# janelia-flyem/flypylib

Measured on AMD Instinct MI355X. Metric: inference Mvoxels/sec, vgg_like (rf 18, 22^3 coarse -> 88^3 per reference tile), synthetic EM uint8 volume, higher is better.
Workload: dtype f16s; 1 GPU; the 520^3 volume of BASELINE.json's metric (configs[0]'s substack size) per GPU: vgg_like inference, 520x520x520 synthetic uint8 volume, reference tile lattice 102^3 (pitch 88), u8 in / f32 out resident in HBM; tile_in=102, executor=vgg_split_f16, parallelism=z-slab tile sharding x1, no collective, device=AMD Radeon Graphics (gfx950:sramecc+:xnack-)

## Files before the change

flypylib_amd/csrc/vgg_plan.h:

```cpp
#pragma once
#include <algorithm>
#include <cstdint>
#include <vector>

struct VggSlab {
  int64_t VZ, VY, VX;
  int64_t fz_hi;
  int64_t cz_lo, cz_hi;
  int CY, CX;
  bool empty;
};

static inline VggSlab vgg_slab(const int64_t dims[3], const std::vector<int32_t> &origins_z,
                               int32_t out_sz_z, int32_t zb, int32_t ze, int off) {
  VggSlab s = {};
  s.VZ = dims[0] - 2 * off; s.VY = dims[1] - 2 * off; s.VX = dims[2] - 2 * off;
  s.empty = s.VZ <= 0 || s.VY <= 0 || s.VX <= 0 || zb >= ze;
  if (s.empty) return s;
  const int64_t fz_lo = (int64_t)origins_z[zb] - off;
  s.fz_hi = std::min<int64_t>((int64_t)origins_z[ze - 1] - off + out_sz_z, s.VZ);
  s.cz_lo = fz_lo / 4; s.cz_hi = (s.fz_hi + 3) / 4;
  s.CY = (int)((s.VY + 3) / 4); s.CX = (int)((s.VX + 3) / 4);
  return s;
}

struct VggPyramid {
  int P2, P1;
  explicit VggPyramid(int64_t C) : P2((int)C + 2), P1(2 * P2 + 2) {}
};
struct Vgg2Pyramid {
  int Q, T3, H;
  explicit Vgg2Pyramid(int64_t C) : Q((int)C + 2), T3(2 * Q + 2), H(T3 + 2) {}
};

static inline int64_t vgg_chunk_rows(int64_t budget_bytes, int64_t bytes_per_fine_row,
                                     int fixed_rows, int64_t span, int64_t cap = 0) {
  int64_t c = std::max<int64_t>(4, (budget_bytes / bytes_per_fine_row - fixed_rows) / 2);
  c = std::min<int64_t>(c, span);
  c = (c + 3) / 4 * 4;
  return cap ? std::min<int64_t>(c, cap) : c;
}

static inline int64_t vgg_split_max_p1_rows(int P1Y, int P1X, int tile_z) {
  return ((int64_t)1 << 32) / 16 / ((int64_t)P1Y * P1X) - (tile_z + 2);
}
static inline int64_t vgg_split_chunk_cap(int64_t max_rows) {
  return std::max<int64_t>(4, ((max_rows - VggPyramid(0).P1) / 2) / 4 * 4);
}

enum { MID_INTERIOR = 0, MID_XCOL = 1, MID_ZLAYER = 2 };

struct MidGeo {
  int BZ, BY, BX;
  int ZS;
  constexpr int TZ() const { return BZ + 2; }
  constexpr int TY() const { return BY + 2; }
  constexpr int TX() const { return BX + 2; }
  constexpr int slots() const { return (TZ() - 1) * ZS + TY() * TX(); }
  constexpr int slot(int tz, int ty, int tx) const { return tz * ZS + ty * TX() + tx; }
};
constexpr MidGeo mid_geo(int o) {
  return o == MID_XCOL ? MidGeo{8, 16, 4, 108} : o == MID_ZLAYER ? MidGeo{4, 8, 16, 182} : MidGeo{8, 4, 16, 118};
}

struct MidVox { int z, y, x; };
constexpr MidVox mid_voxel(int o, int wave, int sub, int c) {
  return o == MID_XCOL     ? MidVox{2 * (wave >> 1) + (sub >> 1), c, 2 * (wave & 1) + (sub & 1)}
         : o == MID_ZLAYER ? MidVox{2 * (wave >> 2) + (sub >> 1), 2 * (wave & 3) + (sub & 1), c}
                           : MidVox{2 * (wave >> 1) + (sub >> 1), 2 * (wave & 1) + (sub & 1), c};
}
constexpr MidVox mid_slot_voxel(const MidGeo &g, int s) {
  const int tz = s / g.ZS < g.TZ() ? s / g.ZS : g.TZ() - 1;
  const int rem = s - tz * g.ZS < g.TY() * g.TX() ? s - tz * g.ZS : g.TY() * g.TX() - 1;
  return MidVox{tz, rem / g.TX(), rem % g.TX()};
}
constexpr int mid_tap_slot(const MidGeo &g, int tap) { return g.slot(tap / 9, (tap / 3) % 3, tap % 3); }

struct MidWalk {
  int nbx, nby, nbz;
  int z0, x0;
  constexpr int64_t blocks() const { return (int64_t)nbx * nby * nbz; }
};
struct MidPlan { MidWalk w[3]; };

static inline MidPlan vgg_mid_plan(int Z, int Y, int X, bool reorient) {
  auto cdiv = [](int a, int b) { return (a + b - 1) / b; };
  const MidGeo gi = mid_geo(MID_INTERIOR), gx = mid_geo(MID_XCOL), gz = mid_geo(MID_ZLAYER);
  MidPlan p = {};
  MidWalk &in = p.w[MID_INTERIOR], &xc = p.w[MID_XCOL], &zl = p.w[MID_ZLAYER];
  in = MidWalk{cdiv(2 * X, gi.BX), cdiv(2 * Y, gi.BY), cdiv(2 * Z, gi.BZ), 0, 0};
  if (!reorient) return p;
  const int live_x = 2 * X % gi.BX, live_z = 2 * Z % gi.BZ;
  if (live_x) {
    const MidWalk c = {cdiv(live_x, gx.BX), cdiv(2 * Y, gx.BY), cdiv(2 * Z, gx.BZ), 0, (in.nbx - 1) * gi.BX};
    if (c.blocks() < (int64_t)in.nby * in.nbz) { xc = c; --in.nbx; }
  }
  if (live_z && in.nbx) {
    const MidWalk c = {in.nbx, cdiv(2 * Y, gz.BY), cdiv(live_z, gz.BZ), (in.nbz - 1) * gi.BZ, 0};
    if (c.blocks() < (int64_t)in.nbx * in.nby) { zl = c; --in.nbz; }
  }
  return p;
}
```

flypylib_amd/csrc/vgg_split.hip:

```cpp
#define FPL_F16 1
#include <algorithm>
#include <cmath>
#include <initializer_list>

#include "fast_paths.h"
#include "mfma_util.h"
#include "pack_weights.h"
#include "vgg_plan.h"
#include <type_traits>
#include "vgg_split_lds.h"
#include "vgg_tiles.h"

namespace {

constexpr int CH = 48;
constexpr int CHP = 24, NPASS = CH / CHP;
constexpr int LO_OFF = CHP * 2;
constexpr int PASS_BYTES = 2 * LO_OFF;
constexpr int VOX = NPASS * PASS_BYTES;
constexpr int KS = (27 * CHP + 31) / 32;
constexpr int KTAB = (KS + 4) / 4 * 4;
constexpr int KTAB_BYTES = 4 * KTAB * 4;
static_assert(CHP % 8 == 0, "a lane's 8 k-slots stay inside one tap");

__host__ __device__ constexpr int64_t chan_off(int ch, int64_t plane) { return (ch / CHP) * plane + (ch % CHP) * 2; }

__device__ __forceinline__ h16x8 pack_relu_split_x(const f32x4 &blk) {
  u32x4 v;
  Pair2 p;
  p = split_pk_relu(blk[0], blk[1]); v[0] = p.hi; v[2] = p.lo;
  p = split_pk_relu(blk[2], blk[3]); v[1] = p.hi; v[3] = p.lo;
  return __builtin_bit_cast(h16x8, v);
}
__device__ __forceinline__ h16x8 pack_relu_split_x(const f32x4 &blk, unsigned &ovf) {
  const h16x8 r = pack_relu_split_x(blk);
  const u32x4 v = __builtin_bit_cast(u32x4, r);
  ovf_note(ovf, pk_max_i16(v[0], v[1]));
  return r;
}

__device__ __forceinline__ f32x4 chain48(const h16x8 (&w)[4], const Frag2 &h01, h16x8 hx, f32x4 acc) {
  acc = mfma16(w[1], h01.hi, acc);
  acc = mfma16(w[0], h01.lo, acc);
  acc = mfma16(w[2], hx, acc);
  acc = mfma16(w[3], hx, acc);
  return mfma16(w[0], h01.hi, acc);
}

__device__ __forceinline__ void store_split12(unsigned char *vox, int64_t plane, int g, const f32x4 (&v)[3],
                                              unsigned &ovf) {
  unsigned hi[6], lo[6];
#pragma unroll
  for (int b = 0; b < 3; ++b) {
    const Pair2 p0 = split_pk(v[b][0], v[b][1], ovf), p1 = split_pk(v[b][2], v[b][3], ovf);
    hi[2 * b] = p0.hi; hi[2 * b + 1] = p1.hi;
    lo[2 * b] = p0.lo; lo[2 * b + 1] = p1.lo;
  }
  unsigned char *d = vox + (g >> 1) * plane + 24 * (g & 1);
  *reinterpret_cast<u32x4_a8 *>(d) = u32x4_a8{hi[0], hi[1], hi[2], hi[3]};
  *reinterpret_cast<u32x2 *>(d + 16) = u32x2{hi[4], hi[5]};
  *reinterpret_cast<u32x4_a8 *>(d + LO_OFF) = u32x4_a8{lo[0], lo[1], lo[2], lo[3]};
  *reinterpret_cast<u32x2 *>(d + LO_OFF + 16) = u32x2{lo[4], lo[5]};
}

constexpr int S_PZ = 4, S_PY = 8, S_PX = 32;
constexpr int S_TZ = 2 * S_PZ + 2, S_TY = 2 * S_PY + 2, S_TX = 2 * S_PX + 2;
constexpr int S_TP = 80;
constexpr int S_TILE = S_TZ * S_TY * S_TP;
constexpr int S_WAVES = 8;
constexpr int S_ROWS = S_TZ * S_TY;
constexpr int S_WROWS = (S_ROWS + S_WAVES - 1) / S_WAVES;
constexpr int S_TASKS = S_PZ * S_PY * 2 / S_WAVES;
constexpr int S_RPT = 3;
static_assert(S_RPT * S_TASKS >= S_WROWS && S_WROWS <= 64, "stem fill schedule");
constexpr int S_SHTAB = 64 * 48;
constexpr int S_SH2 = 4 * 12;
constexpr int S_SMEM = 4 * S_TILE * 2 + 256 * 4 + S_SHTAB * 4 + 2 * S_SH2 * 4;

struct StemSArgs {
  const void *src;
  int64_t SZ, SY, SX;
  int64_t z_hi;
  float mean, sd;
  float c0;
  const float *shtab;
  int64_t p1z0;
  const h16x8 *w1, *w2;
  const float *shift1, *shift2;
  x8::Tensor p1;
  int nbx, nby, nbz;
  int trim;
  unsigned *flag;
  float xlim;
  unsigned char *dump;
};

__device__ __forceinline__ int stem_row_off(int row) {
  return ((row / 3) * S_TY + row % 3) * S_TP;
}

struct StemBlock {
  int px0, py0, pz0;
  int64_t gz0, gy0, gx0;
  unsigned xc;
  bool x_ok;
};

__device__ __forceinline__ StemBlock stem_block(const StemSArgs &a, int q, int lane) {
  StemBlock b;
  const int xb = q % a.nbx, t = q / a.nbx;
  const int yb = t % a.nby, zb = t / a.nby;
  b.px0 = xb * S_PX; b.py0 = yb * S_PY; b.pz0 = zb * S_PZ;
  b.gz0 = 2 * (a.p1z0 + b.pz0); b.gy0 = 2 * (int64_t)b.py0; b.gx0 = 2 * (int64_t)b.px0;
  const int64_t x = b.gx0 + lane;
  b.x_ok = x < a.SX;
  b.xc = (unsigned)(b.x_ok ? x : a.SX - 1);
  return b;
}

__device__ __forceinline__ int stem_row_of(int wrow0, int l) {
  const int r = wrow0 + (l < S_WROWS ? l : S_WROWS - 1);
  return r < S_ROWS ? r : S_ROWS - 1;
}

template <typename SRC>
__device__ __forceinline__ unsigned stem_row_tab(const StemSArgs &a, const StemBlock &b, int wrow0,
                                                 int lane, const SRC *&base) {
  const int row = stem_row_of(wrow0, lane);
  const int64_t z = b.gz0 + row / S_TY, y = b.gy0 + row % S_TY;
  const bool ok = z < a.z_hi && y < a.SY;
  const int64_t zc = z < a.z_hi ? z : a.z_hi - 1, yc = y < a.SY ? y : a.SY - 1;
  const int64_t zb = b.gz0 < a.z_hi ? b.gz0 : a.z_hi - 1, yb = b.gy0 < a.SY ? b.gy0 : a.SY - 1;
  base = (const SRC *)a.src + (zb * a.SY + yb) * a.SX;
  const unsigned rel = (unsigned)(((zc - zb) * a.SY + (yc - yb)) * a.SX);
  return rel | (ok ? 0x80000000u : 0u);
}

template <typename SRC>
struct StemRows {
  SRC v[S_RPT];
  bool ok[S_RPT];
};

template <typename SRC>
__device__ __forceinline__ void stem_load_rows(const SRC *base, unsigned tab, unsigned xc,
                                               int idx0, StemRows<SRC> &r) {
#pragma unroll
  for (int k = 0; k < S_RPT; ++k) {
    const int idx = idx0 + k < S_WROWS ? idx0 + k : S_WROWS - 1;
    const unsigned t = (unsigned)__builtin_amdgcn_readlane((int)tab, idx);
    r.ok[k] = (t >> 31) != 0u;
    r.v[k] = (base + (t & 0x7FFFFFFFu))[xc];
  }
}

template <typename SRC>
__device__ __forceinline__ unsigned stem_norm(const StemSArgs &a, const unsigned *lut, SRC v,
                                              bool ok, unsigned &xmax) {
  unsigned t;
  if (sizeof(SRC) == 1) {
    t = lut[(unsigned)v & 255u];
  } else {
    const float x = ((float)v - a.mean) / a.sd;
    const unsigned ax = __builtin_bit_cast(unsigned, x) & 0x7FFFFFFFu;
    xmax = ax > xmax ? ax : xmax;
    const h16_t h = (h16_t)x;
    t = (unsigned)h16_bits(x) | ((unsigned)h16_bits(x - (float)h) << 16);
  }
  return ok ? t : 0u;
}

struct StemBits { unsigned b[S_RPT]; };

template <typename SRC>
__device__ __forceinline__ void stem_convert_rows(const StemSArgs &a, const StemBlock &b,
                                                  const unsigned *lut, const StemRows<SRC> &r,
                                                  StemBits &o, unsigned &xmax) {
#pragma unroll
  for (int k = 0; k < S_RPT; ++k) o.b[k] = stem_norm<SRC>(a, lut, r.v[k], r.ok[k] && b.x_ok, xmax);
}

template <bool LO>
__device__ __forceinline__ void stem_write_rows(unsigned short *tile, int wrow0, int idx0, int lane,
                                                const StemBits &o) {
#pragma unroll
  for (int k = 0; k < S_RPT; ++k) {
    const int e = stem_row_of(wrow0, idx0 + k) * S_TP + lane;
    tile[e] = (unsigned short)o.b[k];
    if (LO) tile[S_TILE + e] = (unsigned short)(o.b[k] >> 16);
  }
}

template <typename SRC>
struct StemEdge { SRC v[2]; bool ok[2]; };

template <typename SRC>
__device__ __forceinline__ void stem_load_edge(const StemSArgs &a, const StemBlock &b, int wrow0,
                                               int lane, StemEdge<SRC> &e) {
  const int row = stem_row_of(wrow0, lane);
  const int64_t z = b.gz0 + row / S_TY, y = b.gy0 + row % S_TY;
  const bool rok = z < a.z_hi && y < a.SY;
  const int64_t zc = z < a.z_hi ? z : a.z_hi - 1, yc = y < a.SY ? y : a.SY - 1;
  const SRC *rp = (const SRC *)a.src + (zc * a.SY + yc) * a.SX;
#pragma unroll
  for (int j = 0; j < 2; ++j) {
    const int64_t x = b.gx0 + 64 + j;
    e.ok[j] = rok && x < a.SX;
    e.v[j] = rp[x < a.SX ? x : a.SX - 1];
  }
}

template <typename SRC>
__device__ __forceinline__ void stem_store_edge(const StemSArgs &a, unsigned short *tile,
                                                const unsigned *lut, int wrow0, int lane,
                                                const StemEdge<SRC> &e, unsigned &xmax) {
  const int row = stem_row_of(wrow0, lane);
  const unsigned v0 = stem_norm<SRC>(a, lut, e.v[0], e.ok[0], xmax);
  const unsigned v1 = stem_norm<SRC>(a, lut, e.v[1], e.ok[1], xmax);
  *reinterpret_cast<unsigned *>(&tile[row * S_TP + 64]) = (v0 & 0xFFFFu) | (v1 << 16);
  if (sizeof(SRC) != 1)
    *reinterpret_cast<unsigned *>(&tile[S_TILE + row * S_TP + 64]) = (v0 >> 16) | (v1 & 0xFFFF0000u);
}

struct StemTrim {
  int pxs;
  int ntx, nty;
  int nt;
  int mag;
};

__device__ __forceinline__ StemTrim stem_trim(const StemSArgs &a, const StemBlock &b) {
  StemTrim t;
  const int lx = min(S_PX, a.p1.X - b.px0), ly = min(S_PY, a.p1.Y - b.py0), lz = min(S_PZ, a.p1.Z - b.pz0);
  t.pxs = lx > 8 ? 4 : lx > 4 ? 3 : 2;
  const int pyh = 16 >> t.pxs;
  t.ntx = (lx + (1 << t.pxs) - 1) >> t.pxs;
  t.nty = (ly + pyh - 1) / pyh;
  t.nt = lz * t.nty * t.ntx;
  t.mag = (1024 + t.nty - 1) / t.nty;
  return t;
}

__device__ __forceinline__ bool stem_full(const StemSArgs &a, const StemBlock &b) {
  return b.px0 + S_PX <= a.p1.X && b.py0 + S_PY <= a.p1.Y && b.pz0 + S_PZ <= a.p1.Z;
}

extern __shared__ __attribute__((aligned(16))) unsigned char smem[];

template <typename SRC>
__global__ __launch_bounds__(64 * S_WAVES, 2) void vggs_stem_pool(StemSArgs a) {
  unsigned short *tiles = reinterpret_cast<unsigned short *>(smem);
  unsigned *lut = reinterpret_cast<unsigned *>(smem + 4 * S_TILE * 2);
  const int tid = threadIdx.x, lane = tid & 63;
  const int wave = __builtin_amdgcn_readfirstlane(tid >> 6);
  const int c = lane & 15, g = lane >> 4;
  const int nblocks = a.nbx * a.nby * a.nbz;
  int q = blockIdx.x;
  if (q >= nblocks) return;
  constexpr bool INT = sizeof(SRC) == 1;
  if (INT && tid < 256) lut[tid] = (unsigned)h16_bits((float)tid - a.c0);
  const unsigned char *shtab = smem + 4 * S_TILE * 2 + 256 * 4;
  if (INT)
    for (int i = tid; i < S_SHTAB; i += 64 * S_WAVES)
      reinterpret_cast<float *>(smem + 4 * S_TILE * 2 + 256 * 4)[i] = a.shtab[i];

  int offP[2][3], offS[2][2];
#pragma unroll
  for (int e = 0; e < 2; ++e) {
#pragma unroll
    for (int i = 0; i < 3; ++i)
      offP[e][i] = 2 * (g < 3 ? stem_row_off(3 * g + i) + (e == 0 ? 0 : 2)
                              : stem_row_off(6 + i) + (e == 0 ? 2 : 0));
#pragma unroll
    for (int h = 0; h < 2; ++h)
      offS[e][h] = 2 * (stem_row_off(2 * (g < 3 ? g : 2) + h) + (e == 0 ? 2 : 1));
  }
  h16x8 w1[2][2][3], w2[4][3];
  float *sh2t = reinterpret_cast<float *>(smem + 4 * S_TILE * 2 + 256 * 4 + S_SHTAB * 4);
  if (tid < S_SH2) {
    const float v = a.shift2[x8::out_channel((tid % 12) / 4, tid / 12, tid % 4)];
    sh2t[tid] = v;
    sh2t[S_SH2 + tid] = -v;
  }
  const f32x4 *sh2g = reinterpret_cast<const f32x4 *>(sh2t + 12 * g);
  const f32x4 *sh2n = reinterpret_cast<const f32x4 *>(sh2t + S_SH2 + 12 * g);
  f32x4 sh1[3];
#pragma unroll
  for (int p = 0; p < 2; ++p)
#pragma unroll
    for (int s = 0; s < 2; ++s)
#pragma unroll
      for (int b = 0; b < 3; ++b) {
        w1[p][s][b] = a.w1[((p * 2 + s) * 3 + b) * 64 + lane];
        w2[2 * p + s][b] = a.w2[((2 * p + s) * 3 + b) * 64 + lane];
      }
#pragma unroll
  for (int b = 0; b < 3; ++b)
#pragma unroll
    for (int r = 0; r < 4; ++r) {
      sh1[b][r] = a.shift1[16 * b + 4 * g + r];
    }
  __syncthreads();

  unsigned ovf = 0u, xmax = 0u;
  const int wrow0 = wave * S_WROWS;
  StemBlock blk = stem_block(a, q, lane);
  {
    const SRC *base0;
    const unsigned tab0 = stem_row_tab<SRC>(a, blk, wrow0, lane, base0);
    for (int i0 = 0; i0 < S_WROWS; i0 += S_RPT) {
      StemRows<SRC> rr;
      StemBits hb;
      stem_load_rows<SRC>(base0, tab0, blk.xc, i0, rr);
      stem_convert_rows<SRC>(a, blk, lut, rr, hb, xmax);
      stem_write_rows<!INT>(tiles, wrow0, i0, lane, hb);
    }
    StemEdge<SRC> ee;
    stem_load_edge<SRC>(a, blk, wrow0, lane, ee);
    stem_store_edge<SRC>(a, tiles, lut, wrow0, lane, ee, xmax);
  }
  __syncthreads();

  const int G = (int)gridDim.x;
  auto clampq = [&](int qq, int qlast) { return qq < nblocks ? qq : qlast; };
  StemRows<SRC> rr;
  StemEdge<SRC> ee;
  StemBits hb;
  {
    const StemBlock n0 = stem_block(a, clampq(q + G, q), lane);
    const SRC *bn;
    const unsigned tn = stem_row_tab<SRC>(a, n0, wrow0, lane, bn);
    stem_load_rows<SRC>(bn, tn, n0.xc, 0, rr);
    stem_load_edge<SRC>(a, n0, wrow0, lane, ee);
    stem_convert_rows<SRC>(a, n0, lut, rr, hb, xmax);
    stem_load_rows<SRC>(bn, tn, n0.xc, S_RPT, rr);
    const f32x4 z3[3] = {{0.f, 0.f, 0.f, 0.f}, {0.f, 0.f, 0.f, 0.f}, {0.f, 0.f, 0.f, 0.f}};
    __builtin_amdgcn_sched_barrier(0);
    x8::store12_sel(a.p1, 0, g, z3, ovf, false, a.dump);
  }
  struct Gin {
    unsigned p[INT ? 1 : 2][3], s0[INT ? 1 : 2], s1[INT ? 1 : 2];
  };
  struct Geo { int base, xrel, yrel, zrel, pzl, pyl, pxl; bool live; };
  int cur = 0;
  for (;;) {
    const int qn = q + G;
    const bool has_next = qn < nblocks;
    const StemBlock nxt = stem_block(a, has_next ? qn : q, lane);
    const StemBlock nx2 = stem_block(a, clampq(qn + G, has_next ? qn : q), lane);
    const SRC *base_n, *base_2;
    const unsigned tab_n = stem_row_tab<SRC>(a, nxt, wrow0, lane, base_n);
    const unsigned tab_2 = stem_row_tab<SRC>(a, nx2, wrow0, lane, base_2);
    const unsigned char *tb = reinterpret_cast<const unsigned char *>(tiles + cur * 2 * S_TILE);
    unsigned short *tnext = tiles + (cur ^ 1) * 2 * S_TILE;
    auto geo = [&](int ti) {
      Geo t;
      const int task = wave + S_WAVES * ti;
      const int row = task >> 1;
      const int xh = task & 1;
      t.pzl = row / S_PY; t.pyl = row % S_PY; t.pxl = 16 * xh + c; t.live = true;
      t.base = 2 * (((2 * t.pzl) * S_TY + 2 * t.pyl) * S_TP + 2 * (16 * xh + c));
      t.xrel = (int)(blk.gx0 + 2 * (16 * xh + c) + 3 - a.SX);
      t.yrel = (int)(blk.gy0 + 2 * t.pyl + 3 - a.SY);
      t.zrel = (int)(blk.gz0 + 2 * t.pzl + 3 - a.z_hi);
      return t;
    };
    const StemTrim trm = stem_trim(a, blk);
    auto geo_trim = [&](int ti) {
      Geo t;
      int task = wave + S_WAVES * ti;
      t.live = task < trm.nt;
      task = t.live ? task : trm.nt - 1;
      const int r = task >> (trm.ntx - 1), tx = task & (trm.ntx - 1);
      const int tz = (r * trm.mag) >> 10, ty = r - tz * trm.nty;
      t.pzl = tz;
      t.pyl = (ty << (4 - trm.pxs)) + (c >> trm.pxs);
      t.pxl = (tx << trm.pxs) + (c & ((1 << trm.pxs) - 1));
      t.base = 2 * (((2 * t.pzl) * S_TY + 2 * t.pyl) * S_TP + 2 * t.pxl);
      t.xrel = (int)(blk.gx0 + 2 * t.pxl + 3 - a.SX);
      t.yrel = (int)(blk.gy0 + 2 * t.pyl + 3 - a.SY);
      t.zrel = (int)(blk.gz0 + 2 * t.pzl + 3 - a.z_hi);
      return t;
    };
    const bool interior = INT && blk.gx0 + 2 * S_PX + 2 <= a.SX && blk.gy0 + 2 * S_PY + 2 <= a.SY &&
                          blk.gz0 + 2 * S_PZ + 2 <= a.z_hi;
    auto block_pass = [&](auto edge_t, auto trim_t) {
      constexpr bool EDGE = decltype(edge_t)::value, TRIM = decltype(trim_t)::value;
      auto gg = [&](int ti) {
        if constexpr (TRIM) return geo_trim(ti);
        else return geo(ti);
      };
      const int ntask = TRIM ? max(1, (trm.nt - wave + S_WAVES - 1) / S_WAVES) : S_TASKS;
      f32x4 kin[3];
      if (INT && !EDGE) {
#pragma unroll
        for (int b = 0; b < 3; ++b) kin[b] = *reinterpret_cast<const f32x4 *>(shtab + (4 * g) * 4 + 64 * b);
      }
      auto gather = [&](const Geo &t, int sub, Gin &o) {
        const int sp = sub >> 1, e = sub & 1;
        const int so = 2 * ((((sp >> 1) & 1) * S_TY + (sp & 1)) * S_TP);
#pragma unroll
        for (int part = 0; part < (INT ? 1 : 2); ++part) {
          const unsigned char *tp = tb + part * (S_TILE * 2) + t.base + so;
#pragma unroll
          for (int i = 0; i < 3; ++i) o.p[part][i] = *reinterpret_cast<const unsigned *>(tp + offP[e][i]);
          o.s0[part] = *reinterpret_cast<const unsigned short *>(tp + offS[e][0]);
          o.s1[part] = *reinterpret_cast<const unsigned short *>(tp + offS[e][1]);
        }
      };
      auto gather_init = [&](const Geo &t, int sub, f32x4 (&o)[3]) {
        if (INT && EDGE) {
          const int sp = sub >> 1, e = sub & 1;
          const int pzy = 4 * min(max(t.zrel + (sp >> 1), 0), 3) + min(max(t.yrel + (sp & 1), 0), 3);
          const unsigned char *tp = shtab + ((4 * pzy + min(max(t.xrel + e, 0), 3)) * 48 + 4 * g) * 4;
#pragma unroll
          for (int b = 0; b < 3; ++b) o[b] = *reinterpret_cast<const f32x4 *>(tp + 64 * b);
        }
      };
      auto frag = [&](const Gin &gi, int part) {
        const u32x4 raw = {gi.p[part][0], gi.p[part][1], gi.p[part][2], gi.s0[part] | (gi.s1[part] << 16)};
        return __builtin_bit_cast(h16x8, raw);
      };
      constexpr int NC3 = INT ? 6 : 9;
      auto c3 = [&](int i, int e, const f32x4 (&gin)[3], h16x8 bh, h16x8 bl, f32x4 (&o)[3]) {
        const int b = i % 3, grp = i / 3;
        if (grp == 0) o[b] = mfma16(w1[1][e][b], bh, INT ? (EDGE ? gin[b] : kin[b]) : sh1[b]);
        else if (!INT && grp == 1) o[b] = mfma16(w1[0][e][b], bl, o[b]);
        else o[b] = mfma16(w1[0][e][b], bh, o[b]);
      };
      constexpr int NGB = INT ? 2 : 1, DEPTH = NGB + 1;
      Gin Gd[NGB];
      f32x4 gin[3];
      f32x4 a1n[3];
      f32x4 a2[2][3];
      f32x4 poolf[3];
#pragma unroll
      for (int b = 0; b < 3; ++b) poolf[b] = sh2n[b];
#pragma unroll
      for (int e = 0; e < 2; ++e)
#pragma unroll
        for (int b = 0; b < 3; ++b) a2[e][b] = f32x4{0.f, 0.f, 0.f, 0.f};
      {
        const Geo t0 = gg(0);
        gather(t0, 0, Gd[0]);
        gather_init(t0, 0, gin);
        const h16x8 bh = frag(Gd[0], 0), bl = INT ? bh : frag(Gd[0], INT ? 0 : 1);
#pragma unroll
        for (int i = 0; i < NC3; ++i) c3(i, 0, gin, bh, bl, a1n);
        gather_init(t0, 1, gin);
#pragma unroll
        for (int q = 1; q < DEPTH; ++q) gather(t0, q, Gd[q % NGB]);
      }
#pragma unroll 1
      for (int ti = 0; ti < ntask; ++ti) {
        const bool conv2 = ti + 1 >= S_TASKS, load2 = ti + 2 >= S_TASKS;
        const SRC *lbase = load2 ? base_2 : base_n;
        const unsigned ltab = load2 ? tab_2 : tab_n, lxc = load2 ? nx2.xc : nxt.xc;
        const int lidx = S_RPT * ((ti + 2) & (S_TASKS - 1));
        const Geo tg = gg(ti), tn = gg((ti + 1) & (S_TASKS - 1)), tp = gg((ti + S_TASKS - 1) & (S_TASKS - 1));
#pragma unroll
        for (int sub = 0; sub < 8; ++sub) {
          const int sp = sub >> 1, e = sub & 1, en = e ^ 1;
          f32x4 a1[3];
#pragma unroll
          for (int b = 0; b < 3; ++b) a1[b] = a1n[b];
          const Gin &G = Gd[(sub + 1) % NGB];
          const h16x8 bh = frag(G, 0), bl = INT ? bh : frag(G, INT ? 0 : 1);
          float r[12];
          unsigned hi[6], lo[6];
          auto A = [&](int p) {
            r[2 * p] = relu_f32(a1[p >> 1][2 * (p & 1)]);
            r[2 * p + 1] = relu_f32(a1[p >> 1][2 * (p & 1) + 1]);
            hi[p] = cvt_pk_h16(r[2 * p], r[2 * p + 1]);
          };
          auto B = [&](int p) {
            lo[p] = split_lo_pk(r[2 * p], hi[p], r[2 * p + 1]);
          };
          auto PL = [&](int k) {
#pragma unroll
            for (int j = 2 * k; j < 2 * k + 2; ++j)
              poolf[j >> 2][j & 3] = __builtin_fmaxf(__builtin_fmaxf(poolf[j >> 2][j & 3], a2[0][j >> 2][j & 3]),
                                                     a2[1][j >> 2][j & 3]);
          };
          auto c1 = [&](int i) {
            const int b = i % 3, grp = i / 3;
            const u32x4 h0h = {hi[0], hi[1], hi[2], hi[3]}, h0l = {lo[0], lo[1], lo[2], lo[3]};
            const u32x4 hxv = {hi[4], hi[5], lo[4], lo[5]};
            if (grp == 0) a2[e][b] = mfma16(w2[1][b], __builtin_bit_cast(h16x8, h0h), f32x4{0.f, 0.f, 0.f, 0.f});
            if (grp == 1) a2[e][b] = mfma16(w2[0][b], __builtin_bit_cast(h16x8, h0h), a2[e][b]);
            if (grp == 2) a2[e][b] = mfma16(w2[0][b], __builtin_bit_cast(h16x8, h0l), a2[e][b]);
            if (grp == 3) a2[e][b] = mfma16(w2[2][b], __builtin_bit_cast(h16x8, hxv), a2[e][b]);
            if (grp == 4) a2[e][b] = mfma16(w2[3][b], __builtin_bit_cast(h16x8, hxv), a2[e][b]);
          };
#pragma unroll
          for (int s = 0; s < 15; ++s) {
            if (s < 6) c3(s, en, gin, bh, bl, a1n);
            else c1(s - 6);
            if (s < 6 && e == 0) PL(s);
            if (s < 4) A(s);
            else if (s < 8) B(s - 4);
            else if (s < 10) A(s - 4);
            else if (s < 12) B(s - 6);
            __builtin_amdgcn_sched_barrier(0);
          }
          if (sub + DEPTH < 8) gather(tg, sub + DEPTH, Gd[(sub + DEPTH) % NGB]);
          else gather(tn, sub + DEPTH - 8, Gd[(sub + DEPTH) % NGB]);
          if (sub + 2 < 8) gather_init(tg, sub + 2, gin);
          else gather_init(tn, sub + 2 - 8, gin);
#pragma unroll
          for (int i = 6; i < NC3; ++i) c3(i, en, gin, bh, bl, a1n);
#pragma unroll
          for (int i = 9; i < 15; ++i) c1(i);
          if (sub == 0) {
            const int pz = blk.pz0 + tp.pzl, py = blk.py0 + tp.pyl, px = blk.px0 + tp.pxl;
            f32x4 pv[3];
#pragma unroll
            for (int b = 0; b < 3; ++b) pv[b] = poolf[b] + sh2g[b];
            x8::store12_sel(a.p1, a.p1.vox(pz, py, px), g, pv, ovf,
                            ti > 0 && tp.live && pz < a.p1.Z && py < a.p1.Y && px < a.p1.X, a.dump);
#pragma unroll
            for (int b = 0; b < 3; ++b) poolf[b] = sh2n[b];
          }
          if (sub == 3) stem_write_rows<!INT>(tnext, wrow0, S_RPT * ti, lane, hb);
          if (sub == 5) {
#pragma unroll
            for (int k = 0; k < S_RPT; ++k) {
              unsigned t = sizeof(SRC) == 1 ? (unsigned)rr.v[k] : __builtin_bit_cast(unsigned, (float)rr.v[k]);
              asm volatile("" : "+v"(t));
              rr.v[k] = sizeof(SRC) == 1 ? (SRC)t : (SRC)__builtin_bit_cast(float, t);
            }
            stem_convert_rows<SRC>(a, conv2 ? nx2 : nxt, lut, rr, hb, xmax);
          }
          if (sub == 7) stem_load_rows<SRC>(lbase, ltab, lxc, lidx, rr);
          __builtin_amdgcn_sched_barrier(0);
        }
      }
      {
        const Geo t7 = gg(ntask - 1);
#pragma unroll
        for (int b = 0; b < 3; ++b)
#pragma unroll
          for (int r = 0; r < 4; ++r)
            poolf[b][r] = __builtin_fmaxf(__builtin_fmaxf(poolf[b][r], a2[0][b][r]), a2[1][b][r]);
        const int pz = blk.pz0 + t7.pzl, py = blk.py0 + t7.pyl, px = blk.px0 + t7.pxl;
        f32x4 pv[3];
#pragma unroll
        for (int b = 0; b < 3; ++b) pv[b] = poolf[b] + sh2g[b];
        x8::store12_sel(a.p1, a.p1.vox(pz, py, px), g, pv, ovf,
                        t7.live && pz < a.p1.Z && py < a.p1.Y && px < a.p1.X, a.dump);
      }
      if (TRIM && ntask < S_TASKS) {
        stem_write_rows<!INT>(tnext, wrow0, S_RPT * ntask, lane, hb);
        constexpr int FB = INT ? S_TASKS - 1 : 4;
        StemRows<SRC> f8;
        stem_load_rows<SRC>(base_2, tab_2, nx2.xc, 0, f8);
        stem_load_rows<SRC>(base_2, tab_2, nx2.xc, S_RPT, rr);
#pragma unroll
        for (int j0 = 0; j0 < S_TASKS - 1; j0 += FB) {
          StemRows<SRC> fr[FB];
#pragma unroll
          for (int j = 0; j < FB; ++j)
            if (j0 + j < S_TASKS - 1 && ntask + 1 + j0 + j < S_TASKS)
              stem_load_rows<SRC>(base_n, tab_n, nxt.xc, S_RPT * (ntask + 1 + j0 + j), fr[j]);
#pragma unroll
          for (int j = 0; j < FB; ++j)
            if (j0 + j < S_TASKS - 1 && ntask + 1 + j0 + j < S_TASKS) {
              StemBits fb;
              stem_convert_rows<SRC>(a, nxt, lut, fr[j], fb, xmax);
              stem_write_rows<!INT>(tnext, wrow0, S_RPT * (ntask + 1 + j0 + j), lane, fb);
            }
        }
        stem_convert_rows<SRC>(a, nx2, lut, f8, hb, xmax);
      }
    };
    if (a.trim && !stem_full(a, blk)) block_pass(std::true_type{}, std::true_type{});
    else if (interior) block_pass(std::false_type{}, std::false_type{});
    else block_pass(std::true_type{}, std::false_type{});
    if (!has_next) break;
    stem_store_edge<SRC>(a, tnext, lut, wrow0, lane, ee, xmax);
    stem_load_edge<SRC>(a, nx2, wrow0, lane, ee);
    __syncthreads();
    q = qn;
    blk = nxt;
    cur ^= 1;
  }
  ovf_commit(ovf, a.flag, FPL_RANGE_STEM);
  if (!INT && xmax > __builtin_bit_cast(unsigned, a.xlim)) atomicOr(a.flag, FPL_RANGE_INPUT);
}

template <int TY, int TX>
__device__ __forceinline__ unsigned kslot_entry(int idx) {
  const int g = idx / KTAB;
  int s = idx % KTAB;
  s = s < KS ? s : KS - 1;
  const int f0 = 32 * s + 8 * g;
  const int tap = f0 / CHP, ch0 = f0 % CHP;
  if (tap >= 27) return 0u;
  return (unsigned)((((tap / 9) * TY + (tap / 3) % 3) * TX + tap % 3) * PASS_BYTES + ch0 * 2);
}

constexpr int WQ = 2;

template <typename Fill, typename SubOff>
__device__ __forceinline__ void conv3s_kloop_f(Fill fill, unsigned char *tile,
                                               const unsigned *kofftab, const unsigned char *wglobal,
                                               unsigned vbase, SubOff sub_off, f32x4 (&acc)[4][3],
                                               int tid) {
  const int lane = tid & 63, wave = tid >> 6, g = lane >> 4;
  const unsigned *ktab = kofftab + g * KTAB;
#pragma unroll 1
  for (int pass = 0; pass < NPASS; ++pass) {
    if (pass) __syncthreads();
    fill(pass);
    const unsigned char *wl = wglobal + (size_t)pass * KS * 6 * 1024 + lane * 16;
    h16x8 wq[WQ][6];
#pragma unroll
    for (int d = 0; d < WQ; ++d)
#pragma unroll
      for (int f = 0; f < 6; ++f)
        wq[d][f] = *reinterpret_cast<const h16x8 *>(wl + (size_t)(d * 6 + f) * 1024);
    __syncthreads();
    u32x4 kv = *reinterpret_cast<const u32x4 *>(ktab);
    Frag2 bcur[4], bnxt[4];
#pragma unroll
    for (int sub = 0; sub < 4; ++sub) {
      const unsigned char *p = tile + vbase + kv[0] + sub_off(sub);
      bcur[sub].hi = *reinterpret_cast<const h16x8 *>(p);
      bcur[sub].lo = *reinterpret_cast<const h16x8 *>(p + LO_OFF);
    }
#pragma unroll
    for (int s = 0; s < KS; ++s) {
      if ((s + 1) % 4 == 0) kv = *reinterpret_cast<const u32x4 *>(ktab + s + 1);
      const unsigned koff = kv[(s + 1) % 4];
#pragma unroll
      for (int sub = 0; sub < 4; ++sub) {
        const unsigned char *p = tile + vbase + koff + sub_off(sub);
        bnxt[sub].hi = *reinterpret_cast<const h16x8 *>(p);
        bnxt[sub].lo = *reinterpret_cast<const h16x8 *>(p + LO_OFF);
      }
      __builtin_amdgcn_s_setprio(1);
#pragma unroll
      for (int sub = 0; sub < 4; ++sub)
#pragma unroll
        for (int b = 0; b < 3; ++b) acc[sub][b] = mfma16(wq[s % WQ][3 + b], bcur[sub].hi, acc[sub][b]);
#pragma unroll
      for (int sub = 0; sub < 4; ++sub)
#pragma unroll
        for (int b = 0; b < 3; ++b) acc[sub][b] = mfma16(wq[s % WQ][b], bcur[sub].lo, acc[sub][b]);
#pragma unroll
      for (int sub = 0; sub < 4; ++sub)
#pragma unroll
        for (int b = 0; b < 3; ++b) acc[sub][b] = mfma16(wq[s % WQ][b], bcur[sub].hi, acc[sub][b]);
      __builtin_amdgcn_s_setprio(0);
      if (s + WQ < KS) {
#pragma unroll
        for (int f = 0; f < 6; ++f)
          wq[s % WQ][f] = *reinterpret_cast<const h16x8 *>(wl + (size_t)((s + WQ) * 6 + f) * 1024);
      }
#pragma unroll
      for (int sub = 0; sub < 4; ++sub) bcur[sub] = bnxt[sub];
    }
  }
}

template <int TZ, int TY, int TX, typename SubOff>
__device__ __forceinline__ void conv3s_kloop(const unsigned char *act, int AZ, int AY, int AX,
                                             int z0, int y0, int x0, unsigned char *tile,
                                             const unsigned *kofftab, const unsigned char *wglobal,
                                             unsigned vbase, SubOff sub_off, f32x4 (&acc)[4][3],
                                             int tid) {
  const int lane = tid & 63, wave = tid >> 6;
  auto fill = [&](int pass) {
    stage_tile<TZ, TY, TX, PASS_BYTES, PASS_BYTES>(act + (int64_t)pass * AZ * AY * AX * PASS_BYTES, AZ, AY, AX,
                                                   z0, y0, x0, tile, wave, lane);
  };
  conv3s_kloop_f(fill, tile, kofftab, wglobal, vbase, sub_off, acc, tid);
}

constexpr int M_TZ = 6, M_TY = 6, M_TX = 18;
constexpr int M_TILE_BYTES = ((M_TZ * M_TY * M_TX * PASS_BYTES + 1023) / 1024) * 1024;
constexpr int M_SMEM = M_TILE_BYTES + KTAB_BYTES;
static_assert(2 * M_SMEM <= 160 * 1024, "two workgroups must fit one CU");

struct MidXArgs {
  x8::Tensor p1;
  const unsigned char *w3;
  const h16x8 *w4;
  const float *shift3, *shift4;
  x8::Tensor p2;
  x8::Walk walk;
  unsigned *flag;
};

__global__ __launch_bounds__(64 * x8::WAVES, 2) void vggs_mid_pool(MidXArgs a) {
  unsigned *ktab = reinterpret_cast<unsigned *>(smem + 2 * x8::BUF);
  const int tid = threadIdx.x, lane = tid & 63;
  const int wave = __builtin_amdgcn_readfirstlane(tid >> 6);
  const int c = lane & 15, g = lane >> 4;
  x8::ktab_init(ktab, tid);
  const x8::TileDma td = x8::tile_dma_init(wave, lane, a.p1.Y, a.p1.XP, (unsigned)a.p1.part_bytes());
  const int S = (int)gridDim.x >> 3, nbricks = a.walk.bricks();
  const int group = (int)blockIdx.x & 7, slot = (int)blockIdx.x >> 3;
  x8::Cursor cur;
  if (!x8::cursor_first(a.walk, nbricks, group, slot, S, cur)) return;
  const int64_t part = a.p1.part_bytes();
  auto origin = [&](const x8::Cursor &q) {
    return a.p1.p + a.p1.vox(8 * q.bz, 4 * q.by, 16 * q.bx) * 16;
  };
  const int pzl = wave >> 1, pyl = wave & 1;
  const unsigned vb = (unsigned)(((2 * pzl) * x8::ZS + (2 * pyl) * x8::TX + c) * 16);
  auto sub_off = [](int sub) -> unsigned { return (unsigned)((((sub >> 1) & 1) * x8::ZS + (sub & 1) * x8::TX) * 16); };
  unsigned ovf_all = 0u;
  x8::prime(smem, td, origin(cur), part, a.w3, wave, lane);
  for (;;) {
    x8::Cursor nxt = cur;
    const bool has_next = x8::cursor_next(a.walk, slot, S, nxt);
    int zero = 0;
    asm volatile("" : "+s"(zero));
    f32x4 acc[4][3];
#pragma unroll
    for (int b = 0; b < 3; ++b) {
      const f32x4 sh = *reinterpret_cast<const f32x4 *>(a.shift3 + zero + 16 * b + 4 * g);
#pragma unroll
      for (int sub = 0; sub < 4; ++sub) acc[sub][b] = sh;
    }
    x8::conv_block(smem, ktab + 8 * g, td, origin(cur), origin(has_next ? nxt : cur), part, a.w3, vb,
                   sub_off, wave, lane, acc);
    asm volatile("" : "+s"(zero));
    const h16x8 *w4p = a.w4 + zero;
    f32x4 sh4[3];
#pragma unroll
    for (int b = 0; b < 3; ++b)
#pragma unroll
// ... 722 lines not shown
  return true;
}

namespace {

int split2_infer(fpl_ctx *ctx, SplitState *st, const void *src, int src_dtype, float mean, float sd,
                 const int64_t dims[3], const std::vector<int32_t> origins[3],
                 const int32_t out_sz[3], int32_t zb, int32_t ze, float *dst) {
  hipStream_t stream = ctx->stream;
  constexpr int OFF = 10;
  const int64_t SZ = dims[0], SY = dims[1], SX = dims[2];
  const VggSlab s = vgg_slab(dims, origins[0], out_sz[0], zb, ze, OFF);
  if (s.empty) return 0;
  const Vgg2Pyramid py(s.CY), px(s.CX);
  const int64_t h_row = (int64_t)py.H * px.H * VOX, t_row = (int64_t)py.T3 * px.T3 * VOX;
  const int64_t cz_chunk = vgg_chunk_rows(fpl_vgg_scratch_budget(FPL_VGG_SCRATCH_DEFAULT), h_row + t_row,
                                          Vgg2Pyramid(0).H, s.cz_hi - s.cz_lo);
  const Vgg2Pyramid pz_max(cz_chunk);
  FPL_REQUIRE(ctx, (int64_t)py.H * px.H * PASS_BYTES * 8 < ((int64_t)1 << 32),
              "vgg_like2 split path: a %lld x %lld plane is too large for the tile loader's 32-bit "
              "offsets", (long long)SY, (long long)SX);
  DevTemp tmp(ctx);
  unsigned *flag;
  FPL_TRY(fpl_range_flag(ctx, &flag));
  void *h1v, *l3v, *qv;
  FPL_TRY(tmp.alloc((size_t)pz_max.H * h_row, &h1v));
  FPL_TRY(tmp.alloc((size_t)pz_max.T3 * t_row, &l3v));
  FPL_TRY(tmp.alloc((size_t)pz_max.Q * py.Q * px.Q * VOX, &qv));
  const unsigned char *F = st->frags;
  const float *S = st->shifts;
  for (int64_t c0 = s.cz_lo; c0 < s.cz_hi; c0 += cz_chunk) {
    const int CZ = (int)std::min<int64_t>(cz_chunk, s.cz_hi - c0);
    const Vgg2Pyramid pz(CZ);
    {
      V2SArgs a = {};
      a.src = src; a.SZ = SZ; a.SY = SY; a.SX = SX; a.mean = mean; a.sd = sd;
      a.gz0 = 4 * c0;
      a.wstem = (const h16x8 *)(F + st->off_w[0]); a.shstem = S + st->off_s[0];
      if (src_dtype == FPL_U8) {
        a.wstem = (const h16x8 *)st->w1_int; a.shtab = st->shift1_int; a.c0 = st->int_c0;
      }
      a.w = F + st->off_w[1]; a.shift = S + st->off_s[1];
      a.out = (unsigned char *)h1v; a.OZ = pz.H; a.OY = py.H; a.OX = px.H;
      a.flag = flag; a.xlim = st->xlim;
      a.bg = BlockGrid{(int)ceil_div64(px.H, 8), (int)ceil_div64(py.H, 2), (int)ceil_div64(pz.H, 2)};
      TimedLaunch tl(ctx, "vggs2_stem_conv3_pool");
      if (src_dtype == FPL_U8)
        vggs2_conv3<true, true, uint8_t><<<brick_grid_size(a.bg), 256, V2_SMEM, stream>>>(a);
      else
        vggs2_conv3<true, true, float><<<brick_grid_size(a.bg), 256, V2_SMEM, stream>>>(a);
    }
    {
      V2SArgs a = {};
      a.in = (const unsigned char *)h1v; a.IZ = pz.H; a.IY = py.H; a.IX = px.H;
      a.w = F + st->off_w[2]; a.shift = S + st->off_s[2];
      a.out = (unsigned char *)l3v; a.OZ = pz.T3; a.OY = py.T3; a.OX = px.T3;
      a.flag = flag;
      a.bg = BlockGrid{(int)ceil_div64(px.T3, 16), (int)ceil_div64(py.T3, 4), (int)ceil_div64(pz.T3, 4)};
      TimedLaunch tl(ctx, "vggs2_conv3");
      vggs2_conv3<false, false, uint8_t><<<brick_grid_size(a.bg), 256, V2_SMEM, stream>>>(a);
    }
    {
      V2SArgs a = {};
      a.in = (const unsigned char *)l3v; a.IZ = pz.T3; a.IY = py.T3; a.IX = px.T3;
      a.w = F + st->off_w[3]; a.shift = S + st->off_s[3];
      a.out = (unsigned char *)qv; a.OZ = pz.Q; a.OY = py.Q; a.OX = px.Q;
      a.flag = flag;
      a.bg = BlockGrid{(int)ceil_div64(px.Q, 8), (int)ceil_div64(py.Q, 2), (int)ceil_div64(pz.Q, 2)};
      TimedLaunch tl(ctx, "vggs2_conv3_pool");
      vggs2_conv3<false, true, uint8_t><<<brick_grid_size(a.bg), 256, V2_SMEM, stream>>>(a);
    }
    {
      TailSArgs a;
      a.p2 = (const unsigned char *)qv; a.P2Z = pz.Q; a.P2Y = py.Q; a.P2X = px.Q;
      a.w5 = F + st->off_w[4]; a.shift5 = S + st->off_s[4];
      a.CZ = CZ; a.CY = s.CY; a.CX = s.CX;
      a.w6 = F + st->off_w[5]; a.w7 = F + st->off_w[6]; a.w8 = F + st->off_w[7];
      a.shift6 = S + st->off_s[5]; a.shift7 = S + st->off_s[6]; a.bias8 = st->bias8;
      a.dst = dst; a.DY = SY; a.DX = SX; a.gz0 = c0;
      a.VZ = s.fz_hi; a.VY = s.VY; a.VX = s.VX; a.off = OFF;
      a.flag = flag;
      a.bg = BlockGrid{(int)ceil_div64(s.CX, 16), (int)ceil_div64(s.CY, 4), (int)ceil_div64(CZ, 4)};
      TimedLaunch tl(ctx, "vggs_c5_tail");
      vggs_c5_tail_p24<<<brick_grid_size(a.bg), 256, M_SMEM, stream>>>(a);
    }
    FPL_HIP(ctx, hipGetLastError());
  }
  return 0;
}

}

int fpl_split_infer_volume(fpl_ctx *ctx, fpl_program *prog, const void *src, int src_dtype,
                           float mean, float sd, const int64_t dims[3],
                           const std::vector<int32_t> origins[3], const int32_t out_sz[3],
                           int32_t zb, int32_t ze, float *dst) {
  SplitState *st;
  FPL_TRY(split_prepare(ctx, prog, &st));
  if (src_dtype == FPL_U8) FPL_TRY(split_prepare_int(ctx, prog, st, mean, sd));
  if (fpl_vgg_variant(prog) == 2)
    return split2_infer(ctx, st, src, src_dtype, mean, sd, dims, origins, out_sz, zb, ze, dst);
  hipStream_t stream = ctx->stream;
  const int64_t SZ = dims[0], SY = dims[1], SX = dims[2];
  const VggSlab s = vgg_slab(dims, origins[0], out_sz[0], zb, ze, 7);
  if (s.empty) return 0;
  const VggPyramid py(s.CY), px(s.CX);
  const char *edge_env = getenv("FPL_VGG_EDGE_BLOCKS");
  const int edge_blocks = edge_env ? atoi(edge_env) != 0 : 1;
  FPL_REQUIRE(ctx, (int64_t)S_TZ * SY * SX < ((int64_t)1 << 31),
              "vgg split path: a %lld x %lld plane is too large for the stem's 31-bit row "
              "offsets", (long long)SY, (long long)SX);
  const int64_t max_rows = vgg_split_max_p1_rows(py.P1, px.P1, x8::TZ);
  FPL_REQUIRE(ctx, max_rows >= 14,
              "vgg split path: a %lld x %lld plane is too large for the tile loader's 32-bit "
              "offsets", (long long)SY, (long long)SX);
  const int64_t cz_chunk = vgg_chunk_rows(fpl_vgg_scratch_budget(FPL_VGG_SCRATCH_DEFAULT),
                                          (int64_t)py.P1 * px.P1 * VOX, VggPyramid(0).P1, s.cz_hi - s.cz_lo,
                                          vgg_split_chunk_cap(max_rows));
  const VggPyramid pz_max(cz_chunk);
  DevTemp tmp(ctx);
  unsigned *flag;
  FPL_TRY(fpl_range_flag(ctx, &flag));
  x8::Tensor p1 = {nullptr, pz_max.P1, py.P1, px.P1, px.P1}, p2 = {nullptr, pz_max.P2, py.P2, px.P2, px.P2};
  void *p1v, *p2v;
  FPL_TRY(tmp.alloc((size_t)(p1.bytes() + p1.slack_bytes()), &p1v));
  FPL_TRY(tmp.alloc((size_t)(p2.bytes() + p2.slack_bytes()), &p2v));
  void *dumpv;
  FPL_TRY(tmp.alloc(256, &dumpv));
  const unsigned pgrid = (unsigned)std::max(8, ctx->n_cu / 8 * 8);
  const unsigned char *F = st->frags;
  const float *S = st->shifts;
  for (int64_t c0 = s.cz_lo; c0 < s.cz_hi; c0 += cz_chunk) {
    const int CZ = (int)std::min<int64_t>(cz_chunk, s.cz_hi - c0);
    const VggPyramid pz(CZ);
    p1 = x8::Tensor{(unsigned char *)p1v, pz.P1, py.P1, px.P1, px.P1};
    p2 = x8::Tensor{(unsigned char *)p2v, pz.P2, py.P2, px.P2, px.P2};
    FPL_HIP(ctx, hipMemsetAsync(p1.p + p1.bytes(), 0, (size_t)p1.slack_bytes(), stream));
    FPL_HIP(ctx, hipMemsetAsync(p2.p + p2.bytes(), 0, (size_t)p2.slack_bytes(), stream));
    {
      StemSArgs a;
      a.src = src; a.SZ = SZ; a.SY = SY; a.SX = SX; a.mean = mean; a.sd = sd;
      a.p1z0 = 2 * c0;
      a.z_hi = std::min<int64_t>(SZ, 4 * (c0 + CZ) + 14);
      a.w1 = (const h16x8 *)(F + st->off_w[0]);
      a.w2 = (const h16x8 *)(F + st->off_w[1]);
      a.shift1 = S + st->off_s[0]; a.shift2 = S + st->off_s[1];
      a.c0 = 0.f; a.shtab = nullptr;
      if (src_dtype == FPL_U8) {
        a.w1 = (const h16x8 *)st->w1_int; a.shtab = st->shift1_int;
        a.c0 = st->int_c0;
      }
      a.p1 = p1;
      a.flag = flag; a.xlim = st->xlim; a.dump = (unsigned char *)dumpv;
      a.nbx = (int)ceil_div64(px.P1, S_PX); a.nby = (int)ceil_div64(py.P1, S_PY);
      a.nbz = (int)ceil_div64(pz.P1, S_PZ);
      a.trim = edge_blocks;
      const unsigned grid = (unsigned)std::min<int64_t>((int64_t)a.nbx * a.nby * a.nbz,
                                                        (int64_t)ctx->n_cu);
      TimedLaunch tl(ctx, "vggs_stem_pool");
      if (src_dtype == FPL_U8)
        vggs_stem_pool<uint8_t><<<grid, 64 * S_WAVES, S_SMEM, stream>>>(a);
      else
        vggs_stem_pool<float><<<grid, 64 * S_WAVES, S_SMEM, stream>>>(a);
    }
    {
      MidXArgs a;
      a.p1 = p1;
      a.w3 = F + st->off_w[2];
      a.w4 = (const h16x8 *)(F + st->off_w[3]);
      a.shift3 = S + st->off_s[2]; a.shift4 = S + st->off_s[3];
      a.p2 = p2;
      a.flag = flag;
      const MidPlan mp = vgg_mid_plan(pz.P2, py.P2, px.P2, edge_blocks != 0);
      auto walk_of = [&](int o) { return x8::Walk{mp.w[o].nbx, mp.w[o].nby, mp.w[o].nbz}; };
      TimedLaunch tl(ctx, "vggs_mid_pool");
      if (mp.w[MID_INTERIOR].blocks()) {
        a.walk = walk_of(MID_INTERIOR);
        vggs_mid_pool<<<pgrid, 64 * x8::WAVES, x8::SMEM, stream>>>(a);
      }
      for (int o : {MID_XCOL, MID_ZLAYER}) {
        if (!mp.w[o].blocks()) continue;
        MidEdgeArgs e = {a, mp.w[o].z0, mp.w[o].x0};
        e.m.walk = walk_of(o);
        const unsigned egrid = (unsigned)std::min<int64_t>(pgrid, (mp.w[o].blocks() + 7) / 8 * 8);
        if (o == MID_XCOL)
          vggs_mid_pool_edge<MID_XCOL><<<egrid, 64 * x8::WAVES, x8::SMEM, stream>>>(e);
        else
          vggs_mid_pool_edge<MID_ZLAYER><<<egrid, 64 * x8::WAVES, x8::SMEM, stream>>>(e);
      }
    }
    {
      TailXArgs a;
      a.p2 = p2;
      a.w5 = F + st->off_w[4]; a.shift5 = S + st->off_s[4];
      a.CZ = CZ; a.CY = s.CY; a.CX = s.CX;
      a.w6 = F + st->off_w[5]; a.w7 = F + st->off_w[6]; a.w8 = F + st->off_w[7];
      a.shift6 = S + st->off_s[5]; a.shift7 = S + st->off_s[6]; a.bias8 = st->bias8;
      a.dst = dst; a.DY = SY; a.DX = SX; a.gz0 = c0;
      a.VZ = s.fz_hi; a.VY = s.VY; a.VX = s.VX; a.off = 7;
      a.flag = flag;
      a.walk = x8::Walk{(int)ceil_div64(s.CX, 16), (int)ceil_div64(s.CY, 4), (int)ceil_div64(CZ, 8)};
      TimedLaunch tl(ctx, "vggs_c5_tail");
      vggs_c5_tail<<<pgrid, 64 * x8::WAVES, x8::SMEM, stream>>>(a);
    }
    FPL_HIP(ctx, hipGetLastError());
  }
  return 0;
}
```

Measured before the change: 16010 Mvoxels/s.

## Reorder stem blocks full-first and fill trimmed edge tiles with live-only loads

The stem kernel now walks its blocks in a new order: all full interior blocks come first, then the partial x-column, y-row and z-layer edge blocks. When the next block is a trimmed edge block, the tile is prefetched by a new block-wide loader that fetches only the live rows and columns, replacing the per-wave row pipeline and its trailing catch-up fill in the trim path. This is meant to cut redundant loads and normalisation for mostly-empty edge tiles and to simplify the trimmed pass. In exchange it adds a non-pipelined, block-wide fill and changes the block scheduling order, which could hurt overlap at the boundary between full and edge blocks.

```diff
diff --git a/flypylib_amd/csrc/vgg_plan.h b/flypylib_amd/csrc/vgg_plan.h
--- a/flypylib_amd/csrc/vgg_plan.h
+++ b/flypylib_amd/csrc/vgg_plan.h
@@ -101,3 +101,39 @@
   }
   return p;
 }
+
+struct StemWalk {
+  int nbx, nby, nbz;
+  int fx, fy, fz;
+  constexpr int blocks() const { return nbx * nby * nbz; }
+  constexpr int full() const { return fx * fy * fz; }
+};
+struct StemPos { int xb, yb, zb; };
+
+constexpr StemWalk stem_walk(int nbx, int nby, int nbz, bool cut_x, bool cut_y, bool cut_z, bool split) {
+  return StemWalk{nbx, nby, nbz, nbx - (split && cut_x), nby - (split && cut_y), nbz - (split && cut_z)};
+}
+
+constexpr StemPos stem_walk_block(const StemWalk &w, int s) {
+  if (s < w.full()) return StemPos{s % w.fx, s / w.fx % w.fy, s / (w.fx * w.fy)};
+  s -= w.full();
+  const int ncol = (w.nbx - w.fx) * w.nby * w.nbz;
+  if (s < ncol) return StemPos{w.fx, s % w.nby, s / w.nby};
+  s -= ncol;
+  const int nrow = w.fx * (w.nby - w.fy) * w.nbz;
+  if (s < nrow) return StemPos{s % w.fx, w.fy, s / w.fx};
+  s -= nrow;
+  return StemPos{s % w.fx, s / w.fx, w.fz};
+}
+
+struct StemLive {
+  int nz, ny, nx;
+  int cws;
+  int mag;
+  constexpr int rows() const { return nz * ny; }
+  constexpr int row_z(int r) const { return (r * mag) >> 16; }
+};
+constexpr StemLive stem_live_tile(int pz, int py, int px) {
+  return StemLive{2 * pz + 2, 2 * py + 2, 2 * px + 2, 2 * px + 2 <= 16 ? 4 : 2 * px + 2 <= 32 ? 5 : 6,
+                  (65536 + 2 * py + 1) / (2 * py + 2)};
+}
diff --git a/flypylib_amd/csrc/vgg_split.hip b/flypylib_amd/csrc/vgg_split.hip
--- a/flypylib_amd/csrc/vgg_split.hip
+++ b/flypylib_amd/csrc/vgg_split.hip
@@ -88,7 +88,7 @@
   const h16x8 *w1, *w2;
   const float *shift1, *shift2;
   x8::Tensor p1;
-  int nbx, nby, nbz;
+  StemWalk walk;
   int trim;
   unsigned *flag;
   float xlim;
@@ -108,9 +108,8 @@
 
 __device__ __forceinline__ StemBlock stem_block(const StemSArgs &a, int q, int lane) {
   StemBlock b;
-  const int xb = q % a.nbx, t = q / a.nbx;
-  const int yb = t % a.nby, zb = t / a.nby;
-  b.px0 = xb * S_PX; b.py0 = yb * S_PY; b.pz0 = zb * S_PZ;
+  const StemPos p = stem_walk_block(a.walk, q);
+  b.px0 = p.xb * S_PX; b.py0 = p.yb * S_PY; b.pz0 = p.zb * S_PZ;
   b.gz0 = 2 * (a.p1z0 + b.pz0); b.gy0 = 2 * (int64_t)b.py0; b.gx0 = 2 * (int64_t)b.px0;
   const int64_t x = b.gx0 + lane;
   b.x_ok = x < a.SX;
@@ -227,6 +226,7 @@
   int ntx, nty;
   int nt;
   int mag;
+  int lz;
 };
 
 __device__ __forceinline__ StemTrim stem_trim(const StemSArgs &a, const StemBlock &b) {
@@ -238,11 +238,54 @@
   t.nty = (ly + pyh - 1) / pyh;
   t.nt = lz * t.nty * t.ntx;
   t.mag = (1024 + t.nty - 1) / t.nty;
+  t.lz = lz;
   return t;
 }
 
 __device__ __forceinline__ bool stem_full(const StemSArgs &a, const StemBlock &b) {
   return b.px0 + S_PX <= a.p1.X && b.py0 + S_PY <= a.p1.Y && b.pz0 + S_PZ <= a.p1.Z;
+}
+
+template <typename SRC>
+__device__ __forceinline__ void stem_fill_live(const StemSArgs &a, const StemBlock &b, unsigned short *tile,
+                                               const unsigned *lut, int tid, unsigned &xmax) {
+  const StemTrim t = stem_trim(a, b);
+  const StemLive lv = stem_live_tile(t.lz, t.nty << (4 - t.pxs), t.ntx << t.pxs);
+  const SRC *src = (const SRC *)a.src;
+  auto fetch = [&](int r, int col, SRC &v, bool &ok) {
+    const int tz = lv.row_z(r), ty = r - tz * lv.ny;
+    const int64_t z = b.gz0 + tz, y = b.gy0 + ty, x = b.gx0 + col;
+    ok = z < a.z_hi && y < a.SY && x < a.SX;
+    const int64_t zc = z < a.z_hi ? z : a.z_hi - 1, yc = y < a.SY ? y : a.SY - 1, xc = x < a.SX ? x : a.SX - 1;
+    v = src[(zc * a.SY + yc) * a.SX + xc];
+    return (tz * S_TY + ty) * S_TP + col;
+  };
+  auto put = [&](int e, SRC v, bool ok) {
+    const unsigned h = stem_norm<SRC>(a, lut, v, ok, xmax);
+    tile[e] = (unsigned short)h;
+    if (sizeof(SRC) != 1) tile[S_TILE + e] = (unsigned short)(h >> 16);
+  };
+  constexpr int NT = 64 * S_WAVES, NB = 8;
+  const int n = lv.rows() << lv.cws;
+  for (int i0 = tid; i0 - tid < n; i0 += NB * NT) {
+    SRC v[NB];
+    bool ok[NB];
+    int e[NB];
+#pragma unroll
+    for (int k = 0; k < NB; ++k) {
+      const int i = min(i0 + k * NT, n - 1);
+      e[k] = fetch(i >> lv.cws, i & ((1 << lv.cws) - 1), v[k], ok[k]);
+    }
+#pragma unroll
+    for (int k = 0; k < NB; ++k) put(e[k], v[k], ok[k]);
+  }
+  if (lv.nx > 64) {
+    const int i = min(tid, 2 * lv.rows() - 1);
+    SRC v;
+    bool ok;
+    const int e = fetch(i >> 1, 64 + (i & 1), v, ok);
+    put(e, v, ok);
+  }
 }
 
 extern __shared__ __attribute__((aligned(16))) unsigned char smem[];
@@ -254,7 +297,7 @@
   const int tid = threadIdx.x, lane = tid & 63;
   const int wave = __builtin_amdgcn_readfirstlane(tid >> 6);
   const int c = lane & 15, g = lane >> 4;
-  const int nblocks = a.nbx * a.nby * a.nbz;
+  const int nblocks = a.walk.blocks();
   int q = blockIdx.x;
   if (q >= nblocks) return;
   constexpr bool INT = sizeof(SRC) == 1;
@@ -360,7 +403,7 @@
       const int xh = task & 1;
       t.pzl = row / S_PY; t.pyl = row % S_PY; t.pxl = 16 * xh + c; t.live = true;
       t.base = 2 * (((2 * t.pzl) * S_TY + 2 * t.pyl) * S_TP + 2 * (16 * xh + c));
-      t.xrel = (int)(blk.gx0 + 2 * (16 * xh + c) + 3 - a.SX);
+      t.xrel = (int)(blk.gx0 + 3 - a.SX) + 2 * (16 * xh + c);
       t.yrel = (int)(blk.gy0 + 2 * t.pyl + 3 - a.SY);
       t.zrel = (int)(blk.gz0 + 2 * t.pzl + 3 - a.z_hi);
       return t;
@@ -377,7 +420,7 @@
       t.pyl = (ty << (4 - trm.pxs)) + (c >> trm.pxs);
       t.pxl = (tx << trm.pxs) + (c & ((1 << trm.pxs) - 1));
       t.base = 2 * (((2 * t.pzl) * S_TY + 2 * t.pyl) * S_TP + 2 * t.pxl);
-      t.xrel = (int)(blk.gx0 + 2 * t.pxl + 3 - a.SX);
+      t.xrel = (int)(blk.gx0 + 3 - a.SX) + 2 * t.pxl;
       t.yrel = (int)(blk.gy0 + 2 * t.pyl + 3 - a.SY);
       t.zrel = (int)(blk.gz0 + 2 * t.pzl + 3 - a.z_hi);
       return t;
@@ -521,8 +564,8 @@
 #pragma unroll
             for (int b = 0; b < 3; ++b) poolf[b] = sh2n[b];
           }
-          if (sub == 3) stem_write_rows<!INT>(tnext, wrow0, S_RPT * ti, lane, hb);
-          if (sub == 5) {
+          if (!TRIM && sub == 3) stem_write_rows<!INT>(tnext, wrow0, S_RPT * ti, lane, hb);
+          if (!TRIM && sub == 5) {
 #pragma unroll
             for (int k = 0; k < S_RPT; ++k) {
               unsigned t = sizeof(SRC) == 1 ? (unsigned)rr.v[k] : __builtin_bit_cast(unsigned, (float)rr.v[k]);
@@ -531,7 +574,7 @@
             }
             stem_convert_rows<SRC>(a, conv2 ? nx2 : nxt, lut, rr, hb, xmax);
           }
-          if (sub == 7) stem_load_rows<SRC>(lbase, ltab, lxc, lidx, rr);
+          if (!TRIM && sub == 7) stem_load_rows<SRC>(lbase, ltab, lxc, lidx, rr);
           __builtin_amdgcn_sched_barrier(0);
         }
       }
@@ -548,37 +591,21 @@
         for (int b = 0; b < 3; ++b) pv[b] = poolf[b] + sh2g[b];
         x8::store12_sel(a.p1, a.p1.vox(pz, py, px), g, pv, ovf,
                         t7.live && pz < a.p1.Z && py < a.p1.Y && px < a.p1.X, a.dump);
-      }
-      if (TRIM && ntask < S_TASKS) {
-        stem_write_rows<!INT>(tnext, wrow0, S_RPT * ntask, lane, hb);
-        constexpr int FB = INT ? S_TASKS - 1 : 4;
-        StemRows<SRC> f8;
-        stem_load_rows<SRC>(base_2, tab_2, nx2.xc, 0, f8);
-        stem_load_rows<SRC>(base_2, tab_2, nx2.xc, S_RPT, rr);
-#pragma unroll
-        for (int j0 = 0; j0 < S_TASKS - 1; j0 += FB) {
-          StemRows<SRC> fr[FB];
-#pragma unroll
-          for (int j = 0; j < FB; ++j)
-            if (j0 + j < S_TASKS - 1 && ntask + 1 + j0 + j < S_TASKS)
-              stem_load_rows<SRC>(base_n, tab_n, nxt.xc, S_RPT * (ntask + 1 + j0 + j), fr[j]);
-#pragma unroll
-          for (int j = 0; j < FB; ++j)
-            if (j0 + j < S_TASKS - 1 && ntask + 1 + j0 + j < S_TASKS) {
-              StemBits fb;
-              stem_convert_rows<SRC>(a, nxt, lut, fr[j], fb, xmax);
-              stem_write_rows<!INT>(tnext, wrow0, S_RPT * (ntask + 1 + j0 + j), lane, fb);
-            }
-        }
-        stem_convert_rows<SRC>(a, nx2, lut, f8, hb, xmax);
       }
     };
     if (a.trim && !stem_full(a, blk)) block_pass(std::true_type{}, std::true_type{});
     else if (interior) block_pass(std::false_type{}, std::false_type{});
     else block_pass(std::true_type{}, std::false_type{});
     if (!has_next) break;
-    stem_store_edge<SRC>(a, tnext, lut, wrow0, lane, ee, xmax);
-    stem_load_edge<SRC>(a, nx2, wrow0, lane, ee);
+    if (a.trim && q >= a.walk.full()) {
+      int ft = lane, qf = qn;
+      asm volatile("" : "+v"(ft), "+s"(qf));
+      ft += 64 * wave;
+      stem_fill_live<SRC>(a, stem_block(a, qf, 0), tiles + (cur ^ 1) * 2 * S_TILE, lut, ft, xmax);
+    } else {
+      stem_store_edge<SRC>(a, tnext, lut, wrow0, lane, ee, xmax);
+      stem_load_edge<SRC>(a, nx2, wrow0, lane, ee);
+    }
     __syncthreads();
     q = qn;
     blk = nxt;
@@ -1607,11 +1634,10 @@
       }
       a.p1 = p1;
       a.flag = flag; a.xlim = st->xlim; a.dump = (unsigned char *)dumpv;
-      a.nbx = (int)ceil_div64(px.P1, S_PX); a.nby = (int)ceil_div64(py.P1, S_PY);
-      a.nbz = (int)ceil_div64(pz.P1, S_PZ);
+      a.walk = stem_walk((int)ceil_div64(px.P1, S_PX), (int)ceil_div64(py.P1, S_PY), (int)ceil_div64(pz.P1, S_PZ),
+                         px.P1 % S_PX != 0, py.P1 % S_PY != 0, pz.P1 % S_PZ != 0, edge_blocks != 0);
       a.trim = edge_blocks;
-      const unsigned grid = (unsigned)std::min<int64_t>((int64_t)a.nbx * a.nby * a.nbz,
-                                                        (int64_t)ctx->n_cu);
+      const unsigned grid = (unsigned)std::min<int64_t>((int64_t)a.walk.blocks(), (int64_t)ctx->n_cu);
       TimedLaunch tl(ctx, "vggs_stem_pool");
       if (src_dtype == FPL_U8)
         vggs_stem_pool<uint8_t><<<grid, 64 * S_WAVES, S_SMEM, stream>>>(a);
```

New measurement: 16140 Mvoxels/s (median of 6 runs). Within noise of the previous version (+0.8%).
